# WGLab/NanoMod

Measured on AMD Instinct MI355X. Metric: genomic positions/sec (KS + Stouffer), higher is better.
Workload: dtype f32 keys / f64 p-values; 1 GPU; BASELINE.json configs[1]: E. coli 4.6 Mb: 4600000 positions in total (4600000 per GPU), 200 v 200 reads/position, KS + weighted Stouffer window=5; preset=ecoli, positions_total=4600000, positions_per_gpu=4600000, n0=200, n1=200, layout=fixed stride, ties=few, spread_milli=0, outlier_permille=0, rccl_ranks=0, ks_d=float form, bit for bit, parallelism=one GPU, no collective

## Files before the change

### include/nanomod_hip.h

```cpp
#ifndef NANOMOD_HIP_H
#define NANOMOD_HIP_H

#include <stdint.h>

#ifdef __cplusplus
extern "C" {
#endif

#define NMOD_ABI_VERSION 4

enum {
  NMOD_DTYPE_F32 = 0,
  NMOD_DTYPE_I16_MILLI = 1,
  NMOD_DTYPE_F64 = 2
};

enum { NMOD_MEM_HOST = 0, NMOD_MEM_DEVICE = 1 };

enum { NMOD_METHOD_KS = 0, NMOD_METHOD_STOUFFER = 1, NMOD_METHOD_FISHER = 2 };

enum { NMOD_TEST_KS = 1, NMOD_TEST_MWU = 2, NMOD_TEST_WELCH = 4, NMOD_TEST_ALL = 7 };

enum {
  NMOD_STATUS_MWU_ALL_IDENTICAL = 1,
// ... 13 lines not shown
};

#define NMOD_MAX_GROUP 2048
#define NMOD_MAX_RANKED 65535
#define NMOD_MAX_DEEP 16777215
#define NMOD_MAX_NB 64

typedef struct nmod_params {
  int32_t struct_size;
  int32_t device;
  void*   stream;
  int32_t memspace;
  int32_t dtype;
  int32_t tests;
  int32_t method;
  int32_t nb;
  int32_t want_mstd;
  double  weights_dif;
  int64_t stride0;
  int64_t stride1;
  int32_t max_n0;
  int32_t max_n1;
  void*   timer;
  int32_t flags;
  int32_t reserved;
} nmod_params;

#define NMOD_FLAG_KS_RATIONAL_D 1
#define NMOD_FLAG_CHECK_FINITE 2
#define NMOD_FLAG_NO_COUNTING 4
#define NMOD_FLAG_NO_COUNT_WIDE 8
#define NMOD_FLAG_NO_HOST_NARROW 16
#define NMOD_FLAG_DEEP 32

typedef struct nmod_out {
  double* mwu_u;   double* mwu_p;
  double* t_t;     double* t_p;
  double* ks_d;    double* ks_p;
  double* comb_st; double* comb_p;
  double* mean0;   double* std0;
  double* mean1;   double* std1;
  uint8_t* status;
} nmod_out;

int nmod_abi_version(void);
int nmod_device_count(void);
const char* nmod_strerror(int rc);

int64_t nmod_workspace_bytes(const nmod_params* prm, int64_t npos);

int nmod_detect_batch(const nmod_params* prm, int64_t npos,
                      const void* sig0, const int64_t* off0,
                      const void* sig1, const int64_t* off1,
                      const int32_t* run_id,
                      void* workspace, int64_t workspace_bytes,
                      nmod_out* out);

int nmod_host_pipeline_config(int64_t chunk_bytes, int32_t slots, int32_t threads, int32_t mode);

typedef struct nmod_host_stats {
  int64_t chunks;
  int64_t slots;
  int64_t copy_threads;
  int64_t pinned_input;
  int64_t chunk_positions;
  int64_t device_bytes;
  int64_t pinned_bytes;
  int64_t h2d_bytes;
  int64_t d2h_bytes;
  int64_t narrowed_chunks;
} nmod_host_stats;
int nmod_last_host_stats(nmod_host_stats* st);

typedef struct nmod_dispatch_stats {
  int64_t positions;
  int64_t ks_rank;
  int64_t rank_hist;
  int64_t rank_hist_wide;
  int64_t rank_pair;
  int64_t rank_count;
// ... 111 lines not shown
```

### nanomod_amd/_lib.py

```python
from __future__ import annotations

import ctypes as C
import os

_HERE = os.path.dirname(os.path.abspath(__file__))
LIB_PATH = os.environ.get('NMOD_HIP_LIB') or os.path.join(_HERE, 'libnanomod_hip.so')

NMOD_ABI_VERSION = 4
DTYPE_F32, DTYPE_I16_MILLI, DTYPE_F64 = 0, 1, 2
MEM_HOST, MEM_DEVICE = 0, 1
METHOD_KS, METHOD_STOUFFER, METHOD_FISHER = 0, 1, 2
TEST_KS, TEST_MWU, TEST_WELCH, TEST_ALL = 1, 2, 4, 7
FLAG_KS_RATIONAL_D, FLAG_CHECK_FINITE, FLAG_NO_COUNTING, FLAG_NO_COUNT_WIDE, FLAG_NO_HOST_NARROW = 1, 2, 4, 8, 16
FLAG_DEEP = 32
STATUS_MWU_ALL_IDENTICAL, STATUS_T_NAN, STATUS_EMPTY, STATUS_TOO_LARGE, STATUS_NONFINITE = 1, 2, 4, 8, 16
KERNEL_RANK_STATS, KERNEL_FINALIZE, KERNEL_COMBINE, KERNEL_SYNTH = 0, 1, 2, 3
MAX_GROUP = 2048
MAX_RANKED = 65535
MAX_DEEP = 2 ** 24 - 1
MAX_NB = 64
COMM_ID_BYTES = 128
ERR_NO_RCCL, ERR_RCCL = -6, -7

METHOD_BY_NAME = {'ks': METHOD_KS, 'stouffer': METHOD_STOUFFER, 'fisher': METHOD_FISHER}

OUT_FIELDS = ('mwu_u', 'mwu_p', 't_t', 't_p', 'ks_d', 'ks_p', 'comb_st', 'comb_p',
              'mean0', 'std0', 'mean1', 'std1')


class NmodParams(C.Structure):
    _fields_ = [('struct_size', C.c_int32), ('device', C.c_int32), ('stream', C.c_void_p),
                ('memspace', C.c_int32), ('dtype', C.c_int32), ('tests', C.c_int32),
                ('method', C.c_int32), ('nb', C.c_int32), ('want_mstd', C.c_int32),
                ('weights_dif', C.c_double), ('stride0', C.c_int64), ('stride1', C.c_int64),
                ('max_n0', C.c_int32), ('max_n1', C.c_int32), ('timer', C.c_void_p), ('flags', C.c_int32), ('reserved', C.c_int32)]


class NmodOut(C.Structure):
    _fields_ = [(name, C.c_void_p) for name in OUT_FIELDS] + [('status', C.c_void_p)]


class NmodHostStats(C.Structure):
    _fields_ = [(n, C.c_int64) for n in ('chunks', 'slots', 'copy_threads', 'pinned_input', 'chunk_positions',
                                         'device_bytes', 'pinned_bytes', 'h2d_bytes', 'd2h_bytes', 'narrowed_chunks')]


class NmodDispatchStats(C.Structure):
# ... 6 lines not shown
    check(load().nmod_last_dispatch_stats(C.byref(st)), 'nmod_last_dispatch_stats')
    return {n: int(getattr(st, n)) for n, _ in NmodDispatchStats._fields_ if n != 'reserved'}


FDR_BH, FDR_BY = 0, 1
FDR_BY_NAME = {'bh': FDR_BH, 'by': FDR_BY}


class NmodFdrSummary(C.Structure):
    _fields_ = [('tested', C.c_int64), ('excluded', C.c_int64), ('rejected', C.c_int64), ('p_crit', C.c_double)]


MIX_EQUAL_VAR, MIX_FREE_VAR = 0, 1
MIX_BY_NAME = {'equal': MIX_EQUAL_VAR, 'free': MIX_FREE_VAR}
MIX_NOT_CONVERGED, MIX_DEGENERATE, MIX_SKIPPED, MIX_VAR_FLOORED, MIX_TOO_LARGE = 1, 2, 4, 8, 16
MIX_FIELDS = ('pi', 'mu_mod', 'sd_mod', 'llr')


class NmodMixOut(C.Structure):
    _fields_ = [(name, C.c_void_p) for name in MIX_FIELDS] + [('iters', C.c_void_p), ('status', C.c_void_p), ('resp', C.c_void_p)]


class NanomodLibraryError(RuntimeError):
    pass


_lib = None

_SIGNATURES = {
    'nmod_abi_version': (C.c_int, []),
    'nmod_device_count': (C.c_int, []),
    'nmod_strerror': (C.c_char_p, [C.c_int]),
    'nmod_workspace_bytes': (C.c_int64, [C.POINTER(NmodParams), C.c_int64]),
    'nmod_detect_batch': (C.c_int, [C.POINTER(NmodParams), C.c_int64, C.c_void_p, C.c_void_p, C.c_void_p,
                                    C.c_void_p, C.c_void_p, C.c_void_p, C.c_int64, C.POINTER(NmodOut)]),
    'nmod_combine_track': (C.c_int, [C.POINTER(NmodParams), C.c_int64, C.c_void_p, C.c_void_p, C.c_void_p,
                                     C.c_void_p, C.c_void_p]),
    'nmod_synth_fill': (C.c_int, [C.POINTER(NmodParams), C.c_uint64, C.c_int64, C.c_int64, C.c_int32,
                                  C.c_int32, C.c_int64, C.c_float, C.c_void_p]),
    'nmod_synth_fill_csr': (C.c_int, [C.POINTER(NmodParams), C.c_uint64, C.c_int64, C.c_int64, C.c_int32,
                                      C.c_void_p, C.c_int64, C.c_float, C.c_void_p]),
    'nmod_synth_fill_events': (C.c_int, [C.POINTER(NmodParams), C.c_uint64, C.c_int64, C.c_int64, C.c_int32, C.c_int32,
                                         C.c_void_p, C.c_int64, C.c_int32, C.c_int32, C.c_int32, C.c_void_p]),
    'nmod_evtimer_create': (C.c_int, [C.c_int32, C.POINTER(C.c_void_p)]),
    'nmod_evtimer_reset': (C.c_int, [C.c_void_p]),
    'nmod_evtimer_read': (C.c_int, [C.c_void_p, C.c_int32, C.POINTER(C.c_double), C.POINTER(C.c_int32)]),
    'nmod_evtimer_destroy': (C.c_int, [C.c_void_p]),
    'nmod_selftest': (C.c_int, [C.c_int32]),
    'nmod_comm_unique_id': (C.c_int, [C.c_void_p]),
    'nmod_comm_init_rank': (C.c_int, [C.c_void_p, C.c_int32, C.c_int32, C.c_int32, C.POINTER(C.c_void_p)]),
    'nmod_allgather_tracks': (C.c_int, [C.c_void_p, C.c_void_p, C.c_int64, C.c_int32, C.POINTER(C.c_void_p), C.POINTER(C.c_void_p)]),
    'nmod_comm_destroy': (C.c_int, [C.c_void_p]),
    'nmod_narrow_probe': (C.c_int, [C.c_void_p, C.c_int64, C.c_void_p]),
    'nmod_format_probe': (C.c_int, [C.POINTER(C.c_double), C.c_int64, C.c_int32, C.c_char_p, C.c_int64]),
    'nmod_trim_scratch': (C.c_int, [C.c_int32]),
    'nmod_host_pipeline_config': (C.c_int, [C.c_int64, C.c_int32, C.c_int32, C.c_int32]),
    'nmod_last_host_stats': (C.c_int, [C.POINTER(NmodHostStats)]),
    'nmod_last_dispatch_stats': (C.c_int, [C.POINTER(NmodDispatchStats)]),
    'nmod_build_info': (C.c_char_p, []),
    'nmod_downsample_ks': (C.c_int, [C.POINTER(NmodParams), C.c_int64, C.c_void_p, C.c_void_p, C.c_void_p, C.c_void_p, C.c_void_p, C.c_void_p,
                                     C.c_int32, C.c_double, C.c_uint64, C.c_void_p, C.c_void_p]),
    'nmod_argsort_keys': (C.c_int, [C.POINTER(NmodParams), C.c_int64, C.c_void_p, C.c_void_p]),
    'nmod_describe_dispatch': (C.c_int, [C.POINTER(NmodParams), C.c_int64, C.c_int64, C.c_char_p, C.c_int32]),
    'nmod_write_sign_test': (C.c_int, [C.c_char_p, C.c_int64, C.c_void_p, C.c_char_p, C.c_int32, C.c_char_p, C.c_void_p,
                                       C.c_char_p] + [C.c_void_p] * 10 + [C.c_int32]),
    'nmod_rank_order': (C.c_int, [C.POINTER(NmodParams), C.c_int64, C.c_void_p, C.c_void_p, C.c_void_p, C.c_int32, C.c_void_p]),
# ... 68 lines not shown
```

### nanomod_amd/csrc/ks_rank.hpp

```cpp
#pragma once
#include <hip/hip_runtime.h>
#include <stdint.h>
#include <type_traits>
#include "rank_stats_packed.hpp"
#include "packed_sort_i16.hpp"

namespace nmod {

static __device__ const float kKsBig4[4] = {3.4028234663852886e38f, 3.4028234663852886e38f, 3.4028234663852886e38f, 3.4028234663852886e38f};
static __device__ const unsigned kKsInf4[4] = {0x7f800000u, 0x7f800000u, 0x7f800000u, 0x7f800000u};
static __device__ const unsigned kKsPad16[4] = {0x7fff7fffu, 0x7fff7fffu, 0x7fff7fffu, 0x7fff7fffu};

__host__ __device__ constexpr bool ks_packed_sort(int R, int LG, int DTYPE) { return DTYPE == 1 && R == 16 && (LG == 8 || LG == 16); }

template <int R, int LG>
struct KsLayout {
  static constexpr int C = R * LG;
  static constexpr int ROW = LG + 1;
  static constexpr int REGION = R * ROW;
  static constexpr int LAST = (R - 1) * ROW + LG - 1;
  static constexpr int END = LG;
  __device__ static __forceinline__ int word(int i) { return __mul24(i & (R - 1), ROW) + i / R; }
};

__host__ __device__ constexpr int ks_rank_pos_words(int R, int LG) {
  int w = 2 * R * (LG + 1);
  if (LG <= 16) while ((w & 31) != LG) ++w;
  return w;
}

template <typename T>
__device__ __forceinline__ T ks_global_load(const void* p) {
  typedef const T __attribute__((address_space(1)))* GlobalPtr;
  return *(GlobalPtr)(p);
}

typedef float KsF4v __attribute__((ext_vector_type(4)));
typedef short KsS4v __attribute__((ext_vector_type(4)));
// ... 252 lines not shown
  const int slot = lane / LG;
  float* keys = lds_all + (wave * PW + slot) * POS_WORDS;
  unsigned* hist = reinterpret_cast<unsigned*>(keys + HIST_OFF);
  const int e0 = gl * R;

  const float inf = __builtin_inff();
  LaneSel sel;
#pragma unroll
  for (int b = 0; b < 6; ++b) sel.s[b] = ((lane >> b) & 1) ? inf : -inf;
  for (int r = gl; r < R; r += LG) keys[r * ROW + Lay::END] = inf;
  const bool uniform = args.stride0 > 0 && args.stride1 > 0;
  double* recip = reinterpret_cast<double*>(lds_all + kWavesPerBlock * PW * POS_WORDS);
  if (uniform && threadIdx.x == 0) {
    const int64_t a0 = args.stride0 < args.stride1 ? args.stride0 : args.stride1;
    const int64_t a1 = args.stride0 < args.stride1 ? args.stride1 : args.stride0;
    recip[0] = 1.0 / (double)a0; recip[1] = 1.0 / (double)a1;
  }
  __syncthreads();

  int64_t count = args.npos;
  const int32_t* list = nullptr;
  if (args.alt_gates != nullptr && args.alt_gates[args.class_id] != 0) {
    count = args.alt_meta[args.class_id];
    list = args.alt_list + args.alt_meta[kClassStride + args.class_id];
  } else if (args.pos_list) {
    count = args.class_meta[args.class_id];
    list = args.pos_list + args.class_meta[kClassStride + args.class_id];
  }
  const int64_t items = (count + PW - 1) / PW;
  const int64_t wave_global = (int64_t)blockIdx.x * kWavesPerBlock + wave;
  const int64_t wave_stride = (int64_t)gridDim.x * kWavesPerBlock;

  struct Item { bool valid, swap; int m, q; int64_t pos, off_s, off_q; };
  auto describe = [&](int64_t it) {
    Item d;
    const int64_t li = it * PW + slot;
    d.valid = it < items && li < count;
    d.pos = d.valid ? (list ? (int64_t)list[li] : li) : 0;
    int64_t o0 = 0, o1 = 0; int n0 = 0, n1 = 0;
    if (d.valid) {
      if (args.stride0 > 0) { o0 = (int64_t)((uint64_t)(uint32_t)d.pos * (uint64_t)(uint32_t)args.stride0); n0 = (int)args.stride0; }
      else { o0 = args.off0[d.pos]; n0 = (int)(args.off0[d.pos + 1] - o0); }
      if (args.stride1 > 0) { o1 = (int64_t)((uint64_t)(uint32_t)d.pos * (uint64_t)(uint32_t)args.stride1); n1 = (int)args.stride1; }
      else { o1 = args.off1[d.pos]; n1 = (int)(args.off1[d.pos + 1] - o1); }
    }
    d.swap = n1 < n0;
    d.m = d.swap ? n1 : n0; d.q = d.swap ? n0 : n1;
    d.off_s = d.swap ? o1 : o0; d.off_q = d.swap ? o0 : o1;
    return d;
  };
  const float big = 3.4028234663852886e38f;
  using Q4Raw = typename std::conditional<DTYPE == 0, KsF4, KsS4>::type;
  using Q1Raw = typename std::conditional<DTYPE == 0, float, int16_t>::type;
  auto load_q4 = [&](const void* sig, int64_t off, int idx, bool have) -> Q4Raw {
    using T = Q1Raw;
    const T* src = have ? reinterpret_cast<const T*>(sig) + off + idx : reinterpret_cast<const T*>(kKsBig4);
    return ks_global_load<Q4Raw>(src);
  };
  auto q4_values = [&](float (&xq)[4], const Q4Raw& t, bool have) {
    if constexpr (DTYPE == 0) {
      (void)have;
      xq[0] = t.x; xq[1] = t.y; xq[2] = t.z; xq[3] = t.w;
    } else {
      xq[0] = have ? (float)t.x : big; xq[1] = have ? (float)t.y : big;
      xq[2] = have ? (float)t.z : big; xq[3] = have ? (float)t.w : big;
    }
  };
  auto load_q1 = [&](const void* sig, int64_t off, int idx, bool have) -> Q1Raw {
    using T = Q1Raw;
    return ks_global_load<T>(have ? reinterpret_cast<const T*>(sig) + off + idx : reinterpret_cast<const T*>(kKsBig4));
  };
  auto q1_value = [&](Q1Raw v, bool have) -> float {
    if constexpr (DTYPE == 0) { (void)have; return v; }
    else return have ? (float)v : big;
  };

  Item cur = describe(wave_global);
  constexpr bool PACKED = ks_packed_sort(R, LG, DTYPE);
  float x[R];
  unsigned pk[8];
  {
    KsRows<R, LG, DTYPE> first;
    first.request(cur.swap ? args.sig1 : args.sig0, cur.off_s, cur.m, gl);
    if constexpr (PACKED) first.finish_packed(pk, cur.m, gl);
    else first.finish(x, cur.m, gl);
  }
  __builtin_amdgcn_s_waitcnt(0x0F70);

  for (int64_t it = wave_global; it < items; it += wave_stride) {
    const bool valid = cur.valid;
    const int64_t pos = cur.pos;
    const int m = cur.m, q = cur.q;
    const void* sig_q = cur.swap ? args.sig0 : args.sig1;
    const int64_t off_q = cur.off_q;

    const int full = q / (4 * LG);
    const int tail = (q - full * (4 * LG) + LG - 1) / LG;
    int full_w = full, tail_w = tail;
    if constexpr (PW > 1) {
      full_w = 0; tail_w = 0;
#pragma unroll
      for (int s = 0; s < PW; ++s) {
        full_w = max(full_w, __builtin_amdgcn_readlane(full, s * LG));
        tail_w = max(tail_w, __builtin_amdgcn_readlane(tail, s * LG));
      }
    } else {
      full_w = __builtin_amdgcn_readfirstlane(full);
      tail_w = __builtin_amdgcn_readfirstlane(tail);
    }
    int slots = (full_w * 4 + tail_w) * LG;
    bool coop = false;
    if constexpr (PW > 1) {
      int coop_cost = 0;
#pragma unroll
      for (int sl = 0; sl < PW; ++sl) {
        const int qs = __builtin_amdgcn_readlane(q, sl * LG);
        const int fs = qs / 256;
        coop_cost += fs * 4 + (qs - fs * 256 + 63) / 64;
      }
      coop = coop_cost < full_w * 4 + tail_w;
    }
    const Item nxt = describe(it + wave_stride);
    KsRows<R, LG, DTYPE> rows_next;
    rows_next.request(nxt.swap ? args.sig1 : args.sig0, nxt.off_s, nxt.m, gl);
    constexpr bool PIPE_COOP = LG == 8;
    auto row_of_slot = [&](int sl, const void*& sg, int64_t& of, int& qn) {
      const int src = sl * LG;
      auto rl64 = [&](unsigned long long v) {
        const unsigned lo = (unsigned)__builtin_amdgcn_readlane((int)(unsigned)v, src);
        const unsigned hi = (unsigned)__builtin_amdgcn_readlane((int)(unsigned)(v >> 32), src);
        return ((unsigned long long)hi << 32) | (unsigned long long)lo;
      };
      sg = reinterpret_cast<const void*>((uintptr_t)rl64((unsigned long long)(uintptr_t)sig_q));
      of = (int64_t)rl64((unsigned long long)off_q);
      qn = __builtin_amdgcn_readlane(q, src);
    };
    const void* sig_c = sig_q; int64_t off_c = off_q; int q_c = q;
    int idx_a = 4 * gl, idx_t = full * (4 * LG) + gl;
    bool have_a = !coop && 0 < full, have_t = !coop && idx_t < q;
    if constexpr (PIPE_COOP) {
      if (coop) {
        row_of_slot(0, sig_c, off_c, q_c);
        idx_a = 4 * lane; idx_t = (q_c / 256) * 256 + lane; have_a = q_c >= 256; have_t = idx_t < q_c;
      }
    }
    Q4Raw ra = load_q4(sig_c, off_c, idx_a, have_a);
    Q1Raw rt = load_q1(sig_c, off_c, idx_t, have_t);

    if constexpr (PACKED) {
      seg_sort_packed16<LG>(pk, lane);
      unpack_sorted16<LG>(pk, x);
    } else {
      seg_sort_any<R, LG>(x, sel, lane);
    }
#pragma unroll
// ... 8 lines not shown
    for (int r = 0; r < R; ++r) hist[r * ROW + gl] = 0u;
    if (gl == LG - 1) hist[Lay::END] = 0u;
    __builtin_amdgcn_fence(__ATOMIC_RELEASE, "wavefront");
    __builtin_amdgcn_wave_barrier();

    const bool s_full = __ballot(m == Lay::C) != 0ull;

    auto rank_and_count = [&](auto nv_tag, auto full_tag, const float* kbase, const float* xq) {
      constexpr int NV = decltype(nv_tag)::value;
      constexpr bool FULL = decltype(full_tag)::value;
      const float* lp[NV];
#pragma unroll
      for (int e = 0; e < NV; ++e) lp[e] = ks_search<R, LG, false, FULL>(kbase, xq[e]);
      unsigned inc[NV];
#pragma unroll
      for (int e = 0; e < NV; ++e) inc[e] = (*lp[e] == xq[e]) ? 0x10001u : 0x10000u;
#pragma unroll
      for (int e = 0; e < NV; ++e) atomicAdd(reinterpret_cast<unsigned*>(const_cast<float*>(lp[e])) + HIST_OFF, inc[e]);
    };

    [[maybe_unused]] auto rank_and_count_tops = [&](auto nv_tag, const float* kbase, const KsTops& tops, const float* xq) {
      constexpr int NV = decltype(nv_tag)::value;
      const float* lp[NV];
#pragma unroll
      for (int e = 0; e < NV; ++e) lp[e] = ks_search_tops<R, LG>(kbase, xq[e], tops);
      unsigned inc[NV];
#pragma unroll
      for (int e = 0; e < NV; ++e) inc[e] = (*lp[e] == xq[e]) ? 0x10001u : 0x10000u;
#pragma unroll
      for (int e = 0; e < NV; ++e) atomicAdd(reinterpret_cast<unsigned*>(const_cast<float*>(lp[e])) + HIST_OFF, inc[e]);
    };

    __builtin_amdgcn_s_waitcnt(0x0F70);
    if (!coop) {
#pragma unroll 1
      for (int c = 0; c < full_w; ++c) {
        const Q4Raw rb = load_q4(sig_q, off_q, (c + 1) * (4 * LG) + 4 * gl, c + 1 < full);
        float xa[4];
        q4_values(xa, ra, c < full);
        if (s_full) rank_and_count(std::integral_constant<int, 4>{}, std::true_type{}, keys, xa);
        else rank_and_count(std::integral_constant<int, 4>{}, std::false_type{}, keys, xa);
        ra = rb;
      }
#pragma unroll 1
      for (int c = 0; c < tail_w; ++c) {
        float xq[1] = {q1_value(rt, full * (4 * LG) + c * LG + gl < q)};
        const int idx = full * (4 * LG) + (c + 1) * LG + gl;
        rt = load_q1(sig_q, off_q, idx, idx < q);
        if (s_full) rank_and_count(std::integral_constant<int, 1>{}, std::true_type{}, keys, xq);
        else rank_and_count(std::integral_constant<int, 1>{}, std::false_type{}, keys, xq);
      }
    } else {
      const int cfull = q / 256;
      slots = (cfull * 4 + (q - cfull * 256 + 63) / 64) * 64;
      if constexpr (PIPE_COOP) {
#pragma unroll 1
      for (int sl = 0; sl < PW; ++sl) {
        const void* sig_n = sig_c; int64_t off_n = off_c; int q_n = 0;
        if (sl + 1 < PW) row_of_slot(sl + 1, sig_n, off_n, q_n);
        const int nfs = q_n / 256;
        const Q4Raw na = load_q4(sig_n, off_n, 4 * lane, nfs > 0);
        const Q1Raw nt = load_q1(sig_n, off_n, nfs * 256 + lane, nfs * 256 + lane < q_n);
        const float* kb = lds_all + (wave * PW + sl) * POS_WORDS;
        const int fs = q_c / 256, ts = (q_c - fs * 256 + 63) / 64;
        const KsTops tops = ks_tops<R, LG>(kb);
#pragma unroll 2
// ... 213 lines not shown
```

### nanomod_amd/csrc/nanomod_hip.hip

```cpp
#include <hip/hip_runtime.h>
#include <stdint.h>
#include <string.h>
#include <math.h>
#include <algorithm>
#include <vector>
#include <string>
#include <stdio.h>
#include <atomic>
#include <mutex>
#include <thread>
#include <functional>
#include <condition_variable>
#include <dlfcn.h>

#include "../../include/nanomod_hip.h"
#include "rank_stats.hpp"
#include "rank_stats_launch.hpp"
#include "pvalue_kernels.hpp"
#include "big_rank.hpp"
#include "deep_rank.hpp"
#include "rank_all.hpp"
#include "scratch_pool.hpp"

namespace nmod {

thread_local hipError_t g_last_hip = hipSuccess;
thread_local char g_errbuf[256];

#define NMOD_HIP(call)                                   \
  do {                                                   \
    hipError_t e_ = (call);                              \
    if (e_ != hipSuccess) { g_last_hip = e_; return NMOD_ERR_HIP; } \
  } while (0)

struct EvTimer {
  int capacity;
  std::vector<hipEvent_t> start[NMOD_KERNEL_COUNT], stop[NMOD_KERNEL_COUNT];
  int used[NMOD_KERNEL_COUNT];
};

struct ScopedKernelTimer {
  EvTimer* t; int k; hipStream_t s; int slot;
  ScopedKernelTimer(void* timer, int kernel, hipStream_t stream) : t((EvTimer*)timer), k(kernel), s(stream), slot(-1) {
    if (t && t->used[k] < t->capacity) {
      const hipError_t e = hipEventRecord(t->start[k][t->used[k]], s);
      if (e == hipSuccess) slot = t->used[k]; else g_last_hip = e;
    }
  }
  ~ScopedKernelTimer() {
    if (slot >= 0) {
      const hipError_t e = hipEventRecord(t->stop[k][slot], s);
      if (e == hipSuccess) t->used[k] = slot + 1; else g_last_hip = e;
    }
  }
};

struct Workspace {
  uint32_t* ks_num; uint64_t* mwu_s; uint64_t* tie; double* moments;
  double* tmp_ks_d; double* tmp_ks_p; double* ks_d_ref;
  int32_t* order; int32_t* redo; uint8_t* cls; uint8_t* tied; uint8_t* cnt_done; uint8_t* nonfinite; int32_t* meta;
  int32_t* work_list; int32_t* work_meta;
  unsigned long long* stats;
  int64_t bytes;
};
constexpr int kStatsClass = 8, kStatsGate = 64, kStatsLeft = 128, kStatsTried = 192, kStatsWords = 256;
constexpr int kMetaInts = 256;
constexpr int kMetaMax = 3 * kClassStride;
constexpr int kMetaBigTotal = kMetaMax + 2;
constexpr int kMetaBigCursor = kMetaMax + 4;
constexpr int kMetaWideRedo = kMetaMax + 8;
constexpr int kMetaCntGate = kMetaMax + 10;
constexpr int kMetaDeepTiles = kMetaMax + 12;
constexpr int kMetaRedo = 184;
constexpr int kMetaRedoTotal = 242, kMetaRedoCursor = 244;
static_assert(kMetaRedo + kClassStride < kMetaRedoTotal && kMetaRedoCursor + 2 <= kMetaInts && kMetaBigCursor + 2 <= kMetaWideRedo && kMetaWideRedo < kMetaCntGate && kMetaCntGate < kMetaDeepTiles && kMetaDeepTiles + 2 <= kMetaRedo, "meta layout");
static_assert(kNumPairs <= kClassStride && kStatsClass + kClassStride <= kStatsGate && kStatsGate + kClassStride <= kStatsLeft && kStatsLeft + kClassStride <= kStatsTried && kStatsTried + kClassStride <= kStatsWords, "class tables");

static inline int64_t align256(int64_t x) { return (x + 255) & ~(int64_t)255; }

static Workspace carve(void* base, int64_t npos) {
  Workspace w;
  char* p = (char*)base;
  int64_t o = 0;
  auto take = [&](int64_t bytes) { char* r = p ? p + o : nullptr; o += align256(bytes); return r; };
  w.ks_num = (uint32_t*)take(4 * npos);
  w.mwu_s = (uint64_t*)take(8 * npos);
  w.tie = (uint64_t*)take(8 * npos);
  w.moments = (double*)take(32 * npos);
  w.tmp_ks_d = (double*)take(8 * npos);
  w.tmp_ks_p = (double*)take(8 * npos);
  w.ks_d_ref = (double*)take(8 * npos);
  w.order = (int32_t*)take(4 * npos);
  w.redo = (int32_t*)take(4 * npos);
  w.cls = (uint8_t*)take(npos);
  w.tied = (uint8_t*)take(npos);
  w.cnt_done = (uint8_t*)take(npos + 16);
  w.nonfinite = (uint8_t*)take(npos);
  w.meta = (int32_t*)take(kMetaInts * 4);
  w.work_list = (int32_t*)take(4 * npos);
  w.work_meta = (int32_t*)take(kMetaInts * 4);
  static_assert(3 * kClassStride + 1 + kClassStride <= kMetaInts, "work_meta: counts, offsets, gates, 1 + one class id per probe block");
  w.stats = (unsigned long long*)take(kStatsWords * 8);
  w.bytes = o;
  return w;
}

struct BinArgs {
// ... 207 lines not shown
      }
    }
    if (c == 64 && a.cnt256_ran && a.meta[kMetaCntGate] != 0 && count_of(c256) > 0) { atomicAdd(&a.acc[0], 1ull); atomicAdd(&a.acc[kStatsTried + c256], (unsigned long long)count_of(c256)); }
    if (c == 65 && a.f64) atomicAdd(&a.acc[2], (unsigned long long)a.meta[kMetaRedo]);
  }
  if (a.cnt256_ran && a.meta[kMetaCntGate] != 0) {
    const int64_t n = count_of(c256);
    unsigned mine = 0;
    for (int64_t i = (int64_t)blockIdx.x * 256 + threadIdx.x; i < n; i += (int64_t)gridDim.x * 256) mine += a.cnt_done[i] != 0 ? 1u : 0u;
    mine = (unsigned)wave_sum_u64((unsigned long long)mine);
    if ((threadIdx.x & 63) == 0 && mine) atomicAdd(&a.acc[1], (unsigned long long)mine);
  }
}
struct DispatchRec {
  bool valid = false; bool host = false; int device = 0; hipStream_t stream = nullptr;
  StatsArgs args = {};
  unsigned long long host_totals[kStatsWords] = {};
  int64_t npos = 0;
};
thread_local DispatchRec g_dispatch;
static hipError_t enqueue_dispatch_stats(const StatsArgs& a, hipStream_t stream) {
  const unsigned blocks = a.cnt256_ran ? (unsigned)std::max<int64_t>(1, std::min<int64_t>((a.npos + 255) / 256, 512)) : 1u;
  hipLaunchKernelGGL(dispatch_stats_kernel, dim3(blocks), dim3(256), 0, stream, a);
  return hipGetLastError();
}

static int check_params(const nmod_params* prm) {
  if (!prm || prm->struct_size != (int32_t)sizeof(nmod_params)) return NMOD_ERR_INVALID_ARG;
  if (prm->dtype != NMOD_DTYPE_F32 && prm->dtype != NMOD_DTYPE_I16_MILLI && prm->dtype != NMOD_DTYPE_F64) return NMOD_ERR_INVALID_ARG;
  if (prm->memspace != NMOD_MEM_HOST && prm->memspace != NMOD_MEM_DEVICE) return NMOD_ERR_INVALID_ARG;
  if (prm->method < NMOD_METHOD_KS || prm->method > NMOD_METHOD_FISHER) return NMOD_ERR_INVALID_ARG;
  if (prm->nb < 0 || prm->nb > NMOD_MAX_NB) return NMOD_ERR_INVALID_ARG;
  if ((prm->tests & ~NMOD_TEST_ALL) != 0) return NMOD_ERR_INVALID_ARG;
  if ((prm->flags & ~(NMOD_FLAG_KS_RATIONAL_D | NMOD_FLAG_CHECK_FINITE | NMOD_FLAG_NO_COUNTING | NMOD_FLAG_NO_COUNT_WIDE | NMOD_FLAG_NO_HOST_NARROW | NMOD_FLAG_DEEP)) != 0 || prm->reserved != 0) return NMOD_ERR_INVALID_ARG;
  return NMOD_OK;
}

static int fill_combine_args(const nmod_params* prm, CombineArgs& ca) {
  ca.nb = prm->nb; ca.method = prm->method;
  double dif = prm->weights_dif;
  if (prm->method == NMOD_METHOD_STOUFFER && !(dif > 0.0)) return NMOD_ERR_INVALID_ARG;
  int nb = prm->nb;
  ca.w[nb] = 100.0;
  for (int k = 1; k <= nb; ++k) { ca.w[nb - k] = ca.w[nb - k + 1] / dif; ca.w[nb + k] = ca.w[nb + k - 1] / dif; }
  double ss = 0.0;
  for (int k = 0; k <= 2 * nb; ++k) ss += ca.w[k] * ca.w[k];
  ca.wnorm = sqrt(ss);
  return NMOD_OK;
}

static int launch_combine(const nmod_params* prm, hipStream_t stream, int64_t npos, const double* ks_d,
                          const double* ks_p, const int32_t* run_id, double* comb_st, double* comb_p) {
  CombineArgs ca;
  memset(&ca, 0, sizeof(ca));
  int rc = fill_combine_args(prm, ca);
  if (rc != NMOD_OK) return rc;
  ca.npos = npos; ca.ks_d = ks_d; ca.ks_p = ks_p; ca.run_id = run_id; ca.comb_st = comb_st; ca.comb_p = comb_p;
  unsigned blocks = (unsigned)((npos + kCombineTile - 1) / kCombineTile);
  if (blocks == 0) return NMOD_OK;
  ScopedKernelTimer tm(prm->timer, NMOD_KERNEL_COMBINE, stream);
  hipLaunchKernelGGL(combine_kernel, dim3(blocks), dim3(kCombineTile), 0, stream, ca);
  NMOD_HIP(hipGetLastError());
  return NMOD_OK;
}

constexpr int kMaxDevices = 64;
static std::mutex g_pool_mutex;
// ... 132 lines not shown
    NMOD_HIP(hipStreamSynchronize(stream));
    if (b.max0 <= 0) b.max0 = mx[0];
    if (b.max1 <= 0) b.max1 = mx[1];
  }
  b.deep_flag = (prm->flags & NMOD_FLAG_DEEP) != 0;
  const int64_t group_cap = b.deep_flag ? NMOD_MAX_DEEP : NMOD_MAX_RANKED;
  b.max0 = std::min<int64_t>(b.max0, group_cap); b.max1 = std::min<int64_t>(b.max1, group_cap);
  b.deep_possible = b.deep_flag && std::max(b.max0, b.max1) > NMOD_MAX_RANKED;
  b.deep_dtype = b.f64 ? NMOD_DTYPE_F64 : prm->dtype;
  int cmax0 = size_class_of(std::max<int64_t>(b.max0, 1)), cmax1 = size_class_of(std::max<int64_t>(b.max1, 1));
  b.big_possible = b.all ? (cmax0 >= kNumSizeClasses || cmax1 >= kNumSizeClasses) : (std::min(cmax0, cmax1) >= kNumSizeClasses);
  cmax0 = std::min(cmax0, kNumSizeClasses - 1); cmax1 = std::min(cmax1, kNumSizeClasses - 1);
  b.binned = !(uniform && !b.big_possible && !b.deep_possible);
  if (!meta_cleared && (b.binned || b.f64)) {
    NMOD_HIP(hipMemsetAsync(ws.meta, 0, kMetaInts * 4, stream));
    meta_cleared = true;
  }
  b.rule.lim0 = std::max<int64_t>(b.max0, 1); b.rule.lim1 = std::max<int64_t>(b.max1, 1);
  b.rule.ks_only = b.all ? 0 : 1; b.rule.deep = b.deep_flag ? 1 : 0;
  b.uniform_cls = -1;
  if (!b.binned) {
    b.uniform_cls = classify_position(b.max0, b.max1, b.rule);
    if (b.uniform_cls != 255) b.wanted[b.uniform_cls] = true;
  } else {
    for (int c0 = 0; c0 <= cmax0; ++c0)
      for (int c1 = 0; c1 <= cmax1; ++c1) b.wanted[small_class_of(c0, c1, !b.all)] = true;
  }
  const bool counting_off = (prm->flags & NMOD_FLAG_NO_COUNTING) != 0, cw_off = (prm->flags & NMOD_FLAG_NO_COUNT_WIDE) != 0;
  b.cw_on = !counting_off && !cw_off && (b.all || std::max(b.max0, b.max1) >= kCwKsMinQ);
  const bool wide_f32 = b.all && prm->dtype == NMOD_DTYPE_F32;
  b.wide_redo = wide_f32 && b.big_possible;
  for (int cls = 0; cls < kNumClasses; ++cls) b.wide_redo = b.wide_redo || (wide_f32 && b.wanted[cls] && wide_class(cls));
  if (b.wide_redo && !meta_cleared) NMOD_HIP(hipMemsetAsync(ws.meta + kMetaWideRedo, 0, 4, stream));
  return NMOD_OK;
}

static int enqueue_bins(Batch& b) {
  BinArgs ba;
  ba.npos = b.npos; ba.off0 = b.off0; ba.off1 = b.off1; ba.stride0 = b.stride0; ba.stride1 = b.stride1;
  ba.rule = b.rule; ba.cls = b.ws.cls; ba.meta = b.ws.meta; ba.order = b.ws.order;
  const unsigned blocks = (unsigned)std::min<int64_t>((b.npos + 255) / 256, 4096);
  hipLaunchKernelGGL(classify_kernel, dim3(blocks), dim3(256), 0, b.stream, ba);
  hipLaunchKernelGGL(class_offsets_kernel, dim3(1), dim3(64), 0, b.stream, b.ws.meta);
  hipLaunchKernelGGL(scatter_kernel, dim3((unsigned)((b.npos + kScatterSpan - 1) / kScatterSpan)), dim3(256), 0, b.stream, ba);
  NMOD_HIP(hipGetLastError());
  return NMOD_OK;
}

static int enqueue_k1(Batch& b) {
  const nmod_params* prm = b.prm;
  const Workspace& ws = b.ws;
  RankStatsArgs& ra = b.ra;
  memset(&ra, 0, sizeof(ra));
  ra.sig0 = b.sig0; ra.sig1 = b.sig1; ra.off0 = b.off0; ra.off1 = b.off1; ra.stride0 = b.stride0; ra.stride1 = b.stride1;
  ra.npos = b.npos; ra.ks_num = ws.ks_num; ra.mwu_s = ws.mwu_s; ra.tie = ws.tie; ra.moments = ws.moments; ra.ks_d_ref = ws.ks_d_ref;
  ra.ks_rational_d = (!b.all && (prm->flags & NMOD_FLAG_KS_RATIONAL_D)) ? 1 : 0;
  ra.tied = b.f64 ? ws.tied : nullptr;
  ra.redo_list = ws.redo; ra.redo_count = ws.meta + kMetaWideRedo;
  if (b.binned) { ra.pos_list = ws.order; ra.class_meta = ws.meta; }
  if (b.all && !(prm->flags & NMOD_FLAG_NO_COUNTING)) { ra.cnt_gate = ws.meta + kMetaCntGate; ra.cnt_done = ws.cnt_done; }
  const K1Launcher& k1 = k1_launcher(prm->dtype, b.all);
  CountWideWs cww;
  cww.gates = ws.work_meta + 2 * kClassStride; cww.work_list = ws.work_list; cww.work_meta = ws.work_meta;
  std::vector<int> counted;
  if (b.cw_on) {
    for (int cls = 0; cls < kNumClasses; ++cls) if (b.wanted[cls] && count_wide_class(cls)) counted.push_back(cls);
    if (b.big_possible && b.all) for (int cs = 0; cs < kNumWideBig; ++cs) counted.push_back(kWideBigBase + cs);
  }
  b.cw_ran = !counted.empty();
  if (b.cw_ran) {
    bool vc = false;
    for (int c : counted) vc = vc || class_forms(c).count == kCountValue;
    NMOD_HIP(k1.count_wide_prepare(counted.data(), (int)counted.size(), b.stream, ra, cww));
    NMOD_HIP(k1.count_wide_run(b.num_cus, b.npos, b.stream, ra, cww, vc));
  }
  auto launch_class = [&](int cls, bool cw) -> hipError_t {
    ra.class_id = cls; ra.alt_gates = cw ? cww.gates : nullptr; ra.alt_list = ws.work_list; ra.alt_meta = ws.work_meta;
    const hipError_t e = k1.rank_stats(cls, b.num_cus, b.npos, b.stream, ra);
    ra.alt_gates = nullptr;
    return e;
  };
  for (int cls = 0; cls < kNumClasses; ++cls) if (b.wanted[cls]) NMOD_HIP(launch_class(cls, b.cw_on && count_wide_class(cls)));
  if (b.big_possible && b.all) for (int cs = 0; cs < kNumWideBig; ++cs) NMOD_HIP(launch_class(kWideBigBase + cs, b.cw_on));
  if (b.wide_redo) {
    WideRedoArgs wr;
    wr.sig0 = b.sig0; wr.sig1 = b.sig1; wr.off0 = b.off0; wr.off1 = b.off1; wr.stride0 = b.stride0; wr.stride1 = b.stride1;
    wr.list = ws.redo; wr.count = ws.meta + kMetaWideRedo; wr.tie = ws.tie;
    hipLaunchKernelGGL(wide_redo_kernel, dim3((unsigned)std::min<int64_t>(b.npos, (int64_t)b.num_cus * 2)), dim3(kBigThreads), 0, b.stream, wr);
    NMOD_HIP(hipGetLastError());
  }
  return NMOD_OK;
// ... 385 lines not shown
    if (r_ != 0) { g_last_rccl = r_; g_last_rccl_text = (api)->GetErrorString ? (api)->GetErrorString(r_) : nullptr; return NMOD_ERR_RCCL; } \
  } while (0)
constexpr int kNcclFloat64 = 8;

}
struct nmod_comm { void* comm; int nranks, rank, device; };

extern "C" {

int nmod_abi_version(void) { return NMOD_ABI_VERSION; }

int nmod_device_count(void) {
  int n = 0;
  if (hipGetDeviceCount(&n) != hipSuccess) return 0;
  return n;
}

const char* nmod_strerror(int rc) {
  switch (rc) {
    case NMOD_OK: return "ok";
    case NMOD_ERR_INVALID_ARG: return "invalid argument";
    case NMOD_ERR_HIP:
      snprintf(g_errbuf, sizeof(g_errbuf), "HIP runtime error: %s", hipGetErrorString(g_last_hip));
      return g_errbuf;
    case NMOD_ERR_TOO_LARGE: return "a position has more samples in a group than NMOD_MAX_RANKED (65535; NMOD_MAX_DEEP with NMOD_FLAG_DEEP)";
    case NMOD_ERR_WORKSPACE: return "workspace missing or smaller than nmod_workspace_bytes()";
    case NMOD_ERR_NO_DEVICE: return "no HIP device";
    case NMOD_ERR_NO_RCCL: return "librccl.so could not be bound (neither loaded in this process nor on the loader path)";
    case NMOD_ERR_RCCL:
      snprintf(g_errbuf, sizeof(g_errbuf), "RCCL error %d: %s", g_last_rccl, g_last_rccl_text ? g_last_rccl_text : "?");
      return g_errbuf;
    default: return "unknown error code";
  }
}

int64_t nmod_workspace_bytes(const nmod_params* prm, int64_t npos) {
  (void)prm;
  if (npos < 0) return 0;
  return carve(nullptr, npos).bytes;
}

int nmod_detect_batch(const nmod_params* prm, int64_t npos, const void* sig0, const int64_t* off0,
                      const void* sig1, const int64_t* off1, const int32_t* run_id, void* workspace,
                      int64_t workspace_bytes, nmod_out* out) {
  g_dispatch.valid = false;
  int rc = check_params(prm);
  if (rc != NMOD_OK) return rc;
  if (npos < 0) return NMOD_ERR_INVALID_ARG;
  if (nmod_device_count() <= prm->device || prm->device < 0) return NMOD_ERR_NO_DEVICE;
  NMOD_HIP(hipSetDevice(prm->device));
  DispatchRec rec;
  rec.host = true; rec.npos = npos;
  if (prm->memspace == NMOD_MEM_HOST) {
    rc = detect_host_pipelined(prm, npos, sig0, off0, sig1, off1, run_id, out, rec.host_totals);
  } else {
    rc = prm->dtype == NMOD_DTYPE_F64 ? detect_f64(prm, npos, sig0, off0, sig1, off1, run_id, workspace, workspace_bytes, out, &rec.args)
                                      : detect_device(prm, npos, sig0, off0, sig1, off1, run_id, workspace, workspace_bytes, out, &rec.args);
    if (npos > 0) { rec.host = false; rec.device = prm->device; rec.stream = (hipStream_t)prm->stream; }
  }
  if (rc != NMOD_OK) return rc;
  rec.valid = true;
  g_dispatch = rec;
  return NMOD_OK;
}

int nmod_combine_track(const nmod_params* prm, int64_t npos, const double* ks_d, const double* ks_p,
// ... 563 lines not shown
```

### nanomod_amd/csrc/rank_stats.hpp

```cpp
#pragma once
#include <hip/hip_runtime.h>
#include <stdint.h>
#include "wave_ops.hpp"

namespace nmod {

constexpr int kWavesPerBlock = 4;
constexpr int kLdsPad = 4;
constexpr int kClassStride = 56;

struct RankStatsArgs {
  const void* sig0; const void* sig1;
  const int64_t* off0; const int64_t* off1;
  int64_t stride0, stride1;
  int64_t npos;
  const int32_t* pos_list;
  const int32_t* class_meta;
  int32_t class_id;
  uint32_t* ks_num;
  uint64_t* mwu_s;
  uint64_t* tie;
  double* moments;
  int32_t ks_rational_d;
  double* ks_d_ref;
  uint8_t* tied;
  int32_t* redo_list; int32_t* redo_count;
  int32_t* cnt_gate; uint8_t* cnt_done;
  const int32_t* alt_gates; const int32_t* alt_list; const int32_t* alt_meta;
  int32_t cnt_mode;
};

__device__ __forceinline__ void ce(float& lo, float& hi) {
  float a, b;
  asm("v_min_f32 %0, %2, %3\n\tv_max_f32 %1, %2, %3" : "=&v"(a), "=v"(b) : "v"(lo), "v"(hi));
  lo = a; hi = b;
}

template <int LO, int N, int RR, int R>
__device__ __forceinline__ void oe_merge(float (&x)[R]) {
  constexpr int M = RR * 2;
  if constexpr (M < N) {
    oe_merge<LO, N, M, R>(x);
    oe_merge<LO + RR, N, M, R>(x);
#pragma unroll
    for (int i = LO + RR; i + RR < LO + N; i += M) ce(x[i], x[i + RR]);
  } else {
    ce(x[LO], x[LO + RR]);
  }
}
template <int LO, int N, int R>
__device__ __forceinline__ void oe_sort(float (&x)[R]) {
  if constexpr (N > 1) {
    oe_sort<LO, N / 2, R>(x);
    oe_sort<LO + N / 2, N / 2, R>(x);
    oe_merge<LO, N, 1, R>(x);
  }
}
template <int R>
__device__ __forceinline__ void sort_in_lane(float (&x)[R]) { oe_sort<0, R, R>(x); }

template <int R>
__device__ __forceinline__ void clean_in_lane(float (&x)[R]) {
// ... 100 lines not shown
```

Baseline: 1.308 billion positions/s.

## Add hybrid static/dynamic work claiming for KS rank kernel items

```diff
diff --git a/include/nanomod_hip.h b/include/nanomod_hip.h
--- a/include/nanomod_hip.h
+++ b/include/nanomod_hip.h
@@ -69,6 +69,7 @@
 #define NMOD_FLAG_NO_COUNT_WIDE 8
 #define NMOD_FLAG_NO_HOST_NARROW 16
 #define NMOD_FLAG_DEEP 32
+#define NMOD_FLAG_K1_STATIC_ITEMS 128
 
 typedef struct nmod_out {
   double* mwu_u;   double* mwu_p;
@@ -83,6 +84,8 @@
 int nmod_abi_version(void);
 int nmod_device_count(void);
 const char* nmod_strerror(int rc);
+
+int nmod_item_claim_plan(int64_t items, int64_t waves, int32_t flags, int64_t* plan);
 
 int64_t nmod_workspace_bytes(const nmod_params* prm, int64_t npos);
 
diff --git a/nanomod_amd/_lib.py b/nanomod_amd/_lib.py
--- a/nanomod_amd/_lib.py
+++ b/nanomod_amd/_lib.py
@@ -13,6 +13,7 @@
 TEST_KS, TEST_MWU, TEST_WELCH, TEST_ALL = 1, 2, 4, 7
 FLAG_KS_RATIONAL_D, FLAG_CHECK_FINITE, FLAG_NO_COUNTING, FLAG_NO_COUNT_WIDE, FLAG_NO_HOST_NARROW = 1, 2, 4, 8, 16
 FLAG_DEEP = 32
+FLAG_K1_STATIC_ITEMS = 128
 STATUS_MWU_ALL_IDENTICAL, STATUS_T_NAN, STATUS_EMPTY, STATUS_TOO_LARGE, STATUS_NONFINITE = 1, 2, 4, 8, 16
 KERNEL_RANK_STATS, KERNEL_FINALIZE, KERNEL_COMBINE, KERNEL_SYNTH = 0, 1, 2, 3
 MAX_GROUP = 2048
@@ -85,6 +86,7 @@
     'nmod_device_count': (C.c_int, []),
     'nmod_strerror': (C.c_char_p, [C.c_int]),
     'nmod_workspace_bytes': (C.c_int64, [C.POINTER(NmodParams), C.c_int64]),
+    'nmod_item_claim_plan': (C.c_int, [C.c_int64, C.c_int64, C.c_int32, C.POINTER(C.c_int64)]),
     'nmod_detect_batch': (C.c_int, [C.POINTER(NmodParams), C.c_int64, C.c_void_p, C.c_void_p, C.c_void_p,
                                     C.c_void_p, C.c_void_p, C.c_void_p, C.c_int64, C.POINTER(NmodOut)]),
     'nmod_combine_track': (C.c_int, [C.POINTER(NmodParams), C.c_int64, C.c_void_p, C.c_void_p, C.c_void_p,
diff --git a/nanomod_amd/csrc/item_claim.hpp b/nanomod_amd/csrc/item_claim.hpp
--- /dev/null
+++ b/nanomod_amd/csrc/item_claim.hpp
@@ -0,0 +1,74 @@
+#pragma once
+#include <hip/hip_runtime.h>
+#include <stdint.h>
+
+namespace nmod {
+
+constexpr int kClaimFixedNum = 3, kClaimFixedDen = 8;
+constexpr int kClaimChunkMax = 4;
+constexpr int kClaimItemsPerChunkStep = 32;
+
+template <typename I>
+struct ItemClaimPlanT {
+  I rounds;
+  I first;
+  int32_t chunk;
+  int32_t dynamic;
+};
+using ItemClaimPlan = ItemClaimPlanT<int64_t>;
+
+template <typename I>
+__host__ __device__ inline ItemClaimPlanT<I> item_claim_plan(I items, I waves, bool strided_only) {
+  ItemClaimPlanT<I> p;
+  if (waves < 1) waves = 1;
+  if (strided_only) {
+    p.rounds = (items + waves - 1) / waves; p.first = items; p.chunk = 1; p.dynamic = 0;
+    return p;
+  }
+  const I share = items / waves;
+  p.rounds = share / kClaimFixedDen * kClaimFixedNum + share % kClaimFixedDen * kClaimFixedNum / kClaimFixedDen;
+  p.first = p.rounds * waves;
+  const I c = share / kClaimItemsPerChunkStep;
+  p.chunk = (int32_t)(c < 1 ? 1 : (c > kClaimChunkMax ? kClaimChunkMax : c));
+  p.dynamic = (items - p.first > waves * (I)p.chunk) ? 1 : 0;
+  return p;
+}
+template <typename I>
+__host__ __device__ inline I item_claim_chunk_first(const ItemClaimPlanT<I>& p, I c) { return p.first + c * (I)p.chunk; }
+
+struct ItemWalk {
+  uint32_t step, left, pend, base, chunk;
+  bool dynamic, outstanding;
+  unsigned* counter;
+  unsigned ticket;
+
+  __device__ __forceinline__ uint32_t enter_pending(int lane) {
+    const uint32_t it = pend;
+    step = 1u; left = chunk - 1u;
+    pend = 0xffffffffu;
+    if (dynamic) {
+      if (lane == 0) ticket = atomicInc(counter, 0xffffffffu);
+      outstanding = true;
+    }
+    return it;
+  }
+  __device__ __forceinline__ uint32_t begin(const ItemClaimPlanT<uint32_t>& p, uint32_t wave, uint32_t waves, unsigned* ctr, int lane) {
+    chunk = (uint32_t)p.chunk; dynamic = p.dynamic != 0; outstanding = false; counter = ctr; ticket = 0u;
+    base = item_claim_chunk_first(p, waves);
+    pend = item_claim_chunk_first(p, wave);
+    if (p.rounds > 0u) { step = waves; left = p.rounds - 1u; return wave; }
+    return enter_pending(lane);
+  }
+  __device__ __forceinline__ uint32_t next(uint32_t it, int lane) {
+    if (left > 0u) { --left; return it + step; }
+    return enter_pending(lane);
+  }
+  __device__ __forceinline__ void collect() {
+    if (outstanding) {
+      pend = base + (uint32_t)__builtin_amdgcn_readfirstlane((int)ticket) * chunk;
+      outstanding = false;
+    }
+  }
+};
+
+}
diff --git a/nanomod_amd/csrc/ks_rank.hpp b/nanomod_amd/csrc/ks_rank.hpp
--- a/nanomod_amd/csrc/ks_rank.hpp
+++ b/nanomod_amd/csrc/ks_rank.hpp
@@ -4,6 +4,7 @@
 #include <type_traits>
 #include "rank_stats_packed.hpp"
 #include "packed_sort_i16.hpp"
+#include "item_claim.hpp"
 
 namespace nmod {
 
@@ -322,11 +323,12 @@
   const int64_t wave_stride = (int64_t)gridDim.x * kWavesPerBlock;
 
   struct Item { bool valid, swap; int m, q; int64_t pos, off_s, off_q; };
-  auto describe = [&](int64_t it) {
+  const uint32_t items32 = (uint32_t)items;
+  auto describe = [&](uint32_t it) {
     Item d;
-    const int64_t li = it * PW + slot;
-    d.valid = it < items && li < count;
-    d.pos = d.valid ? (list ? (int64_t)list[li] : li) : 0;
+    const uint32_t li = min(it, items32) * PW + slot;
+    d.valid = li < (uint32_t)count;
+    d.pos = d.valid ? (list ? (int64_t)list[li] : (int64_t)li) : 0;
     int64_t o0 = 0, o1 = 0; int n0 = 0, n1 = 0;
     if (d.valid) {
       if (args.stride0 > 0) { o0 = (int64_t)((uint64_t)(uint32_t)d.pos * (uint64_t)(uint32_t)args.stride0); n0 = (int)args.stride0; }
@@ -365,7 +367,10 @@
     else return have ? (float)v : big;
   };
 
-  Item cur = describe(wave_global);
+  ItemWalk walk;
+  const uint32_t it_first = walk.begin(item_claim_plan<uint32_t>((uint32_t)items, (uint32_t)wave_stride, args.strided_items != 0),
+                                      (uint32_t)wave_global, (uint32_t)wave_stride, args.claim + args.class_id, lane);
+  Item cur = describe(it_first);
   constexpr bool PACKED = ks_packed_sort(R, LG, DTYPE);
   float x[R];
   unsigned pk[8];
@@ -376,8 +381,9 @@
     else first.finish(x, cur.m, gl);
   }
   __builtin_amdgcn_s_waitcnt(0x0F70);
-
-  for (int64_t it = wave_global; it < items; it += wave_stride) {
+  walk.collect();
+
+  for (uint32_t it = it_first, it_next; it < items32; it = it_next) {
     const bool valid = cur.valid;
     const int64_t pos = cur.pos;
     const int m = cur.m, q = cur.q;
@@ -410,7 +416,8 @@
       }
       coop = coop_cost < full_w * 4 + tail_w;
     }
-    const Item nxt = describe(it + wave_stride);
+    it_next = walk.next(it, lane);
+    const Item nxt = describe(it_next);
     KsRows<R, LG, DTYPE> rows_next;
     rows_next.request(nxt.swap ? args.sig1 : args.sig0, nxt.off_s, nxt.m, gl);
     constexpr bool PIPE_COOP = LG == 8;
@@ -485,6 +492,7 @@
     };
 
     __builtin_amdgcn_s_waitcnt(0x0F70);
+    walk.collect();
     if (!coop) {
 #pragma unroll 1
       for (int c = 0; c < full_w; ++c) {
diff --git a/nanomod_amd/csrc/nanomod_hip.hip b/nanomod_amd/csrc/nanomod_hip.hip
--- a/nanomod_amd/csrc/nanomod_hip.hip
+++ b/nanomod_amd/csrc/nanomod_hip.hip
@@ -16,6 +16,7 @@
 #include "../../include/nanomod_hip.h"
 #include "rank_stats.hpp"
 #include "rank_stats_launch.hpp"
+#include "item_claim.hpp"
 #include "pvalue_kernels.hpp"
 #include "big_rank.hpp"
 #include "deep_rank.hpp"
@@ -64,7 +65,7 @@
   int64_t bytes;
 };
 constexpr int kStatsClass = 8, kStatsGate = 64, kStatsLeft = 128, kStatsTried = 192, kStatsWords = 256;
-constexpr int kMetaInts = 256;
+constexpr int kMetaInts = 320;
 constexpr int kMetaMax = 3 * kClassStride;
 constexpr int kMetaBigTotal = kMetaMax + 2;
 constexpr int kMetaBigCursor = kMetaMax + 4;
@@ -73,6 +74,8 @@
 constexpr int kMetaDeepTiles = kMetaMax + 12;
 constexpr int kMetaRedo = 184;
 constexpr int kMetaRedoTotal = 242, kMetaRedoCursor = 244;
+constexpr int kMetaClaim = 256;
+static_assert(kMetaRedoCursor + 2 <= kMetaClaim && kMetaClaim + kClassStride <= kMetaInts, "meta layout: claim counters");
 static_assert(kMetaRedo + kClassStride < kMetaRedoTotal && kMetaRedoCursor + 2 <= kMetaInts && kMetaBigCursor + 2 <= kMetaWideRedo && kMetaWideRedo < kMetaCntGate && kMetaCntGate < kMetaDeepTiles && kMetaDeepTiles + 2 <= kMetaRedo, "meta layout");
 static_assert(kNumPairs <= kClassStride && kStatsClass + kClassStride <= kStatsGate && kStatsGate + kClassStride <= kStatsLeft && kStatsLeft + kClassStride <= kStatsTried && kStatsTried + kClassStride <= kStatsWords, "class tables");
 
@@ -346,7 +349,7 @@
   if (prm->method < NMOD_METHOD_KS || prm->method > NMOD_METHOD_FISHER) return NMOD_ERR_INVALID_ARG;
   if (prm->nb < 0 || prm->nb > NMOD_MAX_NB) return NMOD_ERR_INVALID_ARG;
   if ((prm->tests & ~NMOD_TEST_ALL) != 0) return NMOD_ERR_INVALID_ARG;
-  if ((prm->flags & ~(NMOD_FLAG_KS_RATIONAL_D | NMOD_FLAG_CHECK_FINITE | NMOD_FLAG_NO_COUNTING | NMOD_FLAG_NO_COUNT_WIDE | NMOD_FLAG_NO_HOST_NARROW | NMOD_FLAG_DEEP)) != 0 || prm->reserved != 0) return NMOD_ERR_INVALID_ARG;
+  if ((prm->flags & ~(NMOD_FLAG_KS_RATIONAL_D | NMOD_FLAG_CHECK_FINITE | NMOD_FLAG_NO_COUNTING | NMOD_FLAG_NO_COUNT_WIDE | NMOD_FLAG_NO_HOST_NARROW | NMOD_FLAG_DEEP | NMOD_FLAG_K1_STATIC_ITEMS)) != 0 || prm->reserved != 0) return NMOD_ERR_INVALID_ARG;
   return NMOD_OK;
 }
 
@@ -545,6 +548,7 @@
   b.wide_redo = wide_f32 && b.big_possible;
   for (int cls = 0; cls < kNumClasses; ++cls) b.wide_redo = b.wide_redo || (wide_f32 && b.wanted[cls] && wide_class(cls));
   if (b.wide_redo && !meta_cleared) NMOD_HIP(hipMemsetAsync(ws.meta + kMetaWideRedo, 0, 4, stream));
+  if (!b.all && !meta_cleared && !(prm->flags & NMOD_FLAG_K1_STATIC_ITEMS)) NMOD_HIP(hipMemsetAsync(ws.meta + kMetaClaim, 0, kClassStride * 4, stream));
   return NMOD_OK;
 }
 
@@ -570,6 +574,7 @@
   ra.ks_rational_d = (!b.all && (prm->flags & NMOD_FLAG_KS_RATIONAL_D)) ? 1 : 0;
   ra.tied = b.f64 ? ws.tied : nullptr;
   ra.redo_list = ws.redo; ra.redo_count = ws.meta + kMetaWideRedo;
+  ra.claim = reinterpret_cast<uint32_t*>(ws.meta + kMetaClaim); ra.strided_items = (prm->flags & NMOD_FLAG_K1_STATIC_ITEMS) ? 1 : 0;
   if (b.binned) { ra.pos_list = ws.order; ra.class_meta = ws.meta; }
   if (b.all && !(prm->flags & NMOD_FLAG_NO_COUNTING)) { ra.cnt_gate = ws.meta + kMetaCntGate; ra.cnt_done = ws.cnt_done; }
   const K1Launcher& k1 = k1_launcher(prm->dtype, b.all);
@@ -1021,6 +1026,13 @@
       return g_errbuf;
     default: return "unknown error code";
   }
+}
+
+int nmod_item_claim_plan(int64_t items, int64_t waves, int32_t flags, int64_t* plan) {
+  if (items < 0 || waves < 1 || !plan) return NMOD_ERR_INVALID_ARG;
+  const ItemClaimPlan p = item_claim_plan<int64_t>(items, waves, (flags & NMOD_FLAG_K1_STATIC_ITEMS) != 0);
+  plan[0] = p.rounds; plan[1] = p.first; plan[2] = p.chunk; plan[3] = p.dynamic;
+  return NMOD_OK;
 }
 
 int64_t nmod_workspace_bytes(const nmod_params* prm, int64_t npos) {
diff --git a/nanomod_amd/csrc/rank_stats.hpp b/nanomod_amd/csrc/rank_stats.hpp
--- a/nanomod_amd/csrc/rank_stats.hpp
+++ b/nanomod_amd/csrc/rank_stats.hpp
@@ -28,6 +28,7 @@
   int32_t* cnt_gate; uint8_t* cnt_done;
   const int32_t* alt_gates; const int32_t* alt_list; const int32_t* alt_meta;
   int32_t cnt_mode;
+  uint32_t* claim; int32_t strided_items;
 };
 
 __device__ __forceinline__ void ce(float& lo, float& hi) {
```

Measured after the change: 1.454 billion positions/s, median of 6. 11.2% higher.
